# PaddlePaddle/PaddleFleetX

Measured on AMD Instinct MI355X. Metric: tokens/sec/GPU GPT-3-6.7B pretrain, DP2×TP2×PP2 at 1/2/4/8 MI355X, higher is better.
Workload: dtype bf16; 1 GPU; model=GPT-6.7B, global_batch=32, seq_len=1024, micro_batch=16, parallelism=dp1tp1pp1

## Files before the change

### csrc/bindings.cpp

```cpp
#include <torch/extension.h>

#include <string>
#include <vector>

std::vector<torch::Tensor> layernorm_fwd(torch::Tensor x, torch::Tensor w,
                                         torch::Tensor b, double eps);
std::vector<torch::Tensor> layernorm_bwd(torch::Tensor dy, torch::Tensor x,
                                         torch::Tensor w, torch::Tensor mean,
                                         torch::Tensor rstd);
std::vector<torch::Tensor> rmsnorm_fwd(torch::Tensor x, torch::Tensor w,
                                       double eps);
std::vector<torch::Tensor> rmsnorm_bwd(torch::Tensor dy, torch::Tensor x,
                                       torch::Tensor w, torch::Tensor rstd);
std::vector<torch::Tensor> layernorm_fwd_residual(torch::Tensor x,
                                                  torch::Tensor res,
                                                  torch::Tensor w,
                                                  torch::Tensor b, double eps);
std::vector<torch::Tensor> layernorm_bwd_residual(torch::Tensor dy,
                                                  torch::Tensor x,
                                                  torch::Tensor w,
                                                  torch::Tensor mean,
                                                  torch::Tensor rstd,
                                                  torch::Tensor dsum);
torch::Tensor bias_gelu_fwd(torch::Tensor x, torch::Tensor bias);
std::vector<torch::Tensor> bias_gelu_bwd(torch::Tensor dy, torch::Tensor x,
                                         torch::Tensor bias);
void adamw_flat(torch::Tensor master, torch::Tensor grad, torch::Tensor m,
                torch::Tensor v, torch::Tensor model, double lr, double beta1,
                double beta2, double eps, double wd, long step);
torch::Tensor rope_fwd(torch::Tensor x, torch::Tensor cos, torch::Tensor sin);
torch::Tensor colsum(torch::Tensor x);
void grad_sumsq(torch::Tensor x, torch::Tensor out, long slot);
torch::Tensor softmax_causal_fwd(torch::Tensor s, double scale);
torch::Tensor softmax_causal_bwd(torch::Tensor dy, torch::Tensor y,
                                 double scale);
torch::Tensor softmax_bias_fwd(torch::Tensor s, torch::Tensor bias,
                               long inner, long outer, double scale);
std::vector<torch::Tensor> cross_entropy_fwd(torch::Tensor logits,
// ... 44 lines not shown
                                       torch::Tensor sorted_idx,
                                       torch::Tensor top_p, torch::Tensor u);
std::vector<torch::Tensor> sample_token(
    torch::Tensor logits, torch::Tensor ids_buf, torch::Tensor lens,
    torch::Tensor unfinished, torch::Tensor u, torch::Tensor next_tokens,
    bool greedy, double temperature, long top_k, double top_p,
    double repetition_penalty, long min_length, long eos_token_id,
    long pad_token_id);
std::vector<torch::Tensor> moe_dispatch(torch::Tensor x,
                                        torch::Tensor expert_ids,
                                        long num_experts, long top_k);
torch::Tensor mfma_gemm16_probe(torch::Tensor a, torch::Tensor b);

PYBIND11_MODULE(TORCH_EXTENSION_NAME, m) {
  m.def("layernorm_fwd", &layernorm_fwd, "fused LayerNorm fwd (gfx950)");
  m.def("layernorm_bwd", &layernorm_bwd, "fused LayerNorm bwd");
  m.def("rmsnorm_fwd", &rmsnorm_fwd, "fused RMSNorm fwd");
  m.def("rmsnorm_bwd", &rmsnorm_bwd, "fused RMSNorm bwd");
  m.def("layernorm_fwd_residual", &layernorm_fwd_residual,
        "LN(a+b) fwd, also emits a+b");
  m.def("layernorm_bwd_residual", &layernorm_bwd_residual,
        "LN bwd with fused residual-grad addend");
  m.def("colsum", &colsum, "column sum [N,H] -> fp32 [H] (dbias)");
  m.def("grad_sumsq", &grad_sumsq, "fused sumsq (found_inf + grad norm)");
  m.def("bias_gelu_fwd", &bias_gelu_fwd, "fused bias+gelu fwd");
  m.def("bias_gelu_bwd", &bias_gelu_bwd, "fused bias+gelu bwd");
  m.def("adamw_flat", &adamw_flat, "fused AdamW on flat buffers");
  m.def("rope_fwd", &rope_fwd, "rotary embedding fwd");
  m.def("softmax_causal_fwd", &softmax_causal_fwd,
        "fused scale+causal-mask+softmax fwd");
  m.def("softmax_causal_bwd", &softmax_causal_bwd, "causal softmax bwd");
  m.def("softmax_bias_fwd", &softmax_bias_fwd,
        "fused scale+bias+softmax (gated attention core)");
  m.def("cross_entropy_fwd", &cross_entropy_fwd, "softmax CE fwd");
  m.def("cross_entropy_bwd", &cross_entropy_bwd, "softmax CE bwd");
  m.def("row_max", &row_max, "rowwise max (vocab-parallel CE)");
  m.def("row_sumexp", &row_sumexp, "rowwise sum(exp(x-m))");
// ... 60 lines not shown
```

### csrc/common.h

```cpp
#pragma once

#include <hip/hip_runtime.h>
#include <hip/hip_bf16.h>
#include <hip/hip_fp16.h>

#define WAVE 64
#define DEV_INLINE __device__ __forceinline__

typedef __attribute__((ext_vector_type(2))) short short2v;
typedef __attribute__((ext_vector_type(4))) short short4v;
typedef __attribute__((ext_vector_type(8))) short short8v;
typedef __attribute__((ext_vector_type(4))) float float4v;
typedef __attribute__((ext_vector_type(2))) float float2v;
typedef __attribute__((ext_vector_type(8))) __bf16 bf16x8;
typedef __attribute__((ext_vector_type(4))) __bf16 bf16x4;

typedef __attribute__((ext_vector_type(8))) __bf16 mfma_bf16x8;
typedef __attribute__((ext_vector_type(4))) float mfma_f32x4;

DEV_INLINE float bf2f(__hip_bfloat16 x) { return __bfloat162float(x); }
DEV_INLINE __hip_bfloat16 f2bf(float x) { return __float2bfloat16(x); }

DEV_INLINE float bf_raw2f(unsigned short u) {
  union { unsigned int i; float f; } v;
// ... 142 lines not shown
        ((unsigned short*)&out)[j + 1] = (unsigned short)(u >> 16);
      }
      *reinterpret_cast<short4v*>(p) = out;
    }
  } else {
#pragma unroll
    for (int j = 0; j < VEC; j += 4) {
      float4v out;
#pragma unroll
      for (int k = 0; k < 4; ++k) ((float*)&out)[k] = v[j + k];
      *reinterpret_cast<float4v*>((float*)p + j) = out;
    }
  }
}

#define HIP_CHECK(x)                                                       \
  do {                                                                     \
    hipError_t _e = (x);                                                   \
    if (_e != hipSuccess) {                                                \
      throw std::runtime_error(std::string("HIP error: ") +                \
                               hipGetErrorString(_e));                     \
    }                                                                      \
  } while (0)
```

### csrc/elementwise.hip

```cpp
#include "common.h"
#include "tensor_checks.h"

#include <torch/extension.h>
#include <ATen/hip/HIPContext.h>

namespace {

constexpr int BLOCK = 256;
constexpr float GELU_K = 0.7978845608028654f;

DEV_INLINE float fast_tanh(float y) {
  return 1.f - 2.f / (__expf(2.f * y) + 1.f);
}
DEV_INLINE float gelu_tanh(float x) {
  float t = fast_tanh(GELU_K * (x + 0.044715f * x * x * x));
  return 0.5f * x * (1.f + t);
}
DEV_INLINE float gelu_tanh_grad(float x) {
  float t = fast_tanh(GELU_K * (x + 0.044715f * x * x * x));
  return 0.5f * (1.f + t) +
         0.5f * x * (1.f - t * t) * GELU_K * (1.f + 3.f * 0.044715f * x * x);
}

template <typename T, bool HAS_BIAS, int VEC>
// ... 6 lines not shown
  if constexpr (HAS_BIAS) vload<T, VEC>(bias + col, bv);
  for (long r = blockIdx.y; r < N; r += gridDim.y) {
    const long i = r * H + col;
    float v[VEC];
    vload<T, VEC>(x + i, v);
    float o[VEC];
#pragma unroll
    for (int j = 0; j < VEC; ++j) {
      if constexpr (HAS_BIAS) v[j] += bv[j];
      o[j] = gelu_tanh(v[j]);
    }
    vstore<T, VEC>(y + i, o);
  }
}

template <typename T, bool HAS_BIAS, int VEC>
__global__ __launch_bounds__(BLOCK) void bias_gelu_bwd_kernel(
    const T* __restrict__ dy, const T* __restrict__ x,
    const T* __restrict__ bias, T* __restrict__ dx, long N, int H) {
  const int col = (blockIdx.x * BLOCK + threadIdx.x) * VEC;
  if (col >= H) return;
  float bv[VEC];
  if constexpr (HAS_BIAS) vload<T, VEC>(bias + col, bv);
  for (long r = blockIdx.y; r < N; r += gridDim.y) {
    const long i = r * H + col;
    float v[VEC], d[VEC];
    vload<T, VEC>(x + i, v);
    vload<T, VEC>(dy + i, d);
    float o[VEC];
#pragma unroll
    for (int j = 0; j < VEC; ++j) {
      if constexpr (HAS_BIAS) v[j] += bv[j];
      o[j] = d[j] * gelu_tanh_grad(v[j]);
    }
    vstore<T, VEC>(dx + i, o);
  }
}

template <typename T, int CV>
__global__ __launch_bounds__(BLOCK) void colsum_kernel(
    const T* __restrict__ x, float* __restrict__ out, long N, int H,
    int rows_per_chunk) {
  const int col = (blockIdx.x * BLOCK + threadIdx.x) * CV;
  if (col >= H) return;
  long r0 = (long)blockIdx.y * rows_per_chunk;
  long r1 = r0 + rows_per_chunk < N ? r0 + rows_per_chunk : N;
  float s[CV];
#pragma unroll
  for (int j = 0; j < CV; ++j) s[j] = 0.f;
  for (long r = r0; r < r1; ++r) {
    float v[CV];
    vload<T, CV>(x + r * H + col, v);
#pragma unroll
    for (int j = 0; j < CV; ++j) s[j] += v[j];
  }
#pragma unroll
  for (int j = 0; j < CV; ++j) atomicAdd(&out[col + j], s[j]);
}

template <typename T>
__global__ void grad_sumsq_kernel(const T* __restrict__ x, long n,
                                  float* __restrict__ partial) {
  __shared__ float sred[BLOCK / WAVE];
  float s = 0.f;
  constexpr int V = 4;
  for (long i = ((long)blockIdx.x * BLOCK + threadIdx.x) * V; i < n;
       i += (long)gridDim.x * BLOCK * V) {
    float v[V];
    vload<T, V>(x + i, v);
#pragma unroll
    for (int j = 0; j < V; ++j) s += v[j] * v[j];
  }
// ... 7 lines not shown
  __shared__ double sred[BLOCK / WAVE];
  double s = 0.0;
  for (int i = threadIdx.x; i < np; i += BLOCK) s += (double)partial[i];
#pragma unroll
  for (int off = 32; off > 0; off >>= 1) s += __shfl_xor(s, off, WAVE);
  if (threadIdx.x % WAVE == 0) sred[threadIdx.x / WAVE] = s;
  __syncthreads();
  if (threadIdx.x == 0) {
    double t = 0.0;
#pragma unroll
    for (int w = 0; w < BLOCK / WAVE; ++w) t += sred[w];
    out[slot] = (float)((double)out[slot] + t);
  }
}

void launch_colsum(const void* x, float* out, long N, int H, bool bf16,
                   hipStream_t stream) {
  constexpr int CV = 4;
  int rows_per_chunk = (int)std::max<long>(32, N / 128);
  int nchunks = (int)((N + rows_per_chunk - 1) / rows_per_chunk);
  dim3 grid((H + BLOCK * CV - 1) / (BLOCK * CV), nchunks);
  if (bf16)
    hipLaunchKernelGGL((colsum_kernel<__hip_bfloat16, CV>), grid, dim3(BLOCK),
                       0, stream, (const __hip_bfloat16*)x, out, N, H,
                       rows_per_chunk);
  else
    hipLaunchKernelGGL((colsum_kernel<float, CV>), grid, dim3(BLOCK), 0,
                       stream, (const float*)x, out, N, H, rows_per_chunk);
}

template <typename TM, typename TG>
__global__ void adamw_flat_kernel(float* __restrict__ master,
                                  const TG* __restrict__ grad,
                                  float* __restrict__ m, float* __restrict__ v,
                                  TM* __restrict__ model, long n, float lr,
                                  float beta1, float beta2, float eps,
                                  float wd, float bc1, float bc2) {
  const int VEC = 4;
  for (long i = ((long)blockIdx.x * BLOCK + threadIdx.x) * VEC; i < n;
       i += (long)gridDim.x * BLOCK * VEC) {
    float4v pm = *reinterpret_cast<float4v*>(master + i);
    float4v pg;
    if constexpr (sizeof(TG) == 2) {
// ... 116 lines not shown
                                         torch::Tensor bias) {
  fleetx::check_data(x, "x");
  TORCH_CHECK(x.dim() >= 1, "x must have a last dim");
  fleetx::check_same(dy, x, "dy");
  TORCH_CHECK(dy.sizes() == x.sizes(), "dy must have the shape of x");
  long total = x.numel();
  int H = x.size(-1);
  long N = total / H;
  TORCH_CHECK(H % 4 == 0, "last dim must be divisible by 4");
  bool has_bias = bias.defined() && bias.numel() > 0;
  if (has_bias) {
    fleetx::check_same(bias, x, "bias");
    fleetx::check_numel(bias, H, "bias");
  }
  auto dx = torch::empty_like(x);
  auto stream = at::hip::getCurrentHIPStream();
  bool v8 = H % 8 == 0;
  int vec = v8 ? 8 : 4;
  dim3 grid((H + BLOCK * vec - 1) / (BLOCK * vec),
            (unsigned)std::min<long>(N, 16384));
#define LAUNCH_BG(T, HB, V)                                                  \
  hipLaunchKernelGGL((bias_gelu_bwd_kernel<T, HB, V>), grid, dim3(BLOCK), 0, \
                     stream, (const T*)dy.data_ptr(), (const T*)x.data_ptr(), \
                     has_bias ? (const T*)bias.data_ptr() : nullptr,         \
                     (T*)dx.data_ptr(), N, H)
#define PICK_BG(T, HB) do { if (v8) LAUNCH_BG(T, HB, 8); else LAUNCH_BG(T, HB, 4); } while (0)
  if (x.scalar_type() == torch::kBFloat16) {
    if (has_bias) PICK_BG(__hip_bfloat16, true);
    else PICK_BG(__hip_bfloat16, false);
  } else {
    if (has_bias) PICK_BG(float, true);
    else PICK_BG(float, false);
  }
#undef PICK_BG
#undef LAUNCH_BG
  torch::Tensor db;
  if (has_bias) {
    db = torch::zeros({H}, x.options().dtype(torch::kFloat));
    launch_colsum(dx.data_ptr(), db.data_ptr<float>(), N, H,
                  x.scalar_type() == torch::kBFloat16, stream);
  }
  return {dx, db};
}

void grad_sumsq(torch::Tensor x, torch::Tensor out, long slot) {
  fleetx::check_data(x, "x");
  fleetx::check_aux(out, torch::kFloat, x, "out");
  TORCH_CHECK(slot >= 0 && slot < out.numel(), "slot ", slot,
              " is outside out (", out.numel(), " slots)");
  long n = x.numel();
  TORCH_CHECK(n % 4 == 0, "x.numel() must be divisible by 4");
  if (n == 0) return;
  auto stream = at::hip::getCurrentHIPStream();
  dim3 grid(grid_for(n, BLOCK * 4));
  auto partial = torch::empty({(long)grid.x}, out.options());
// ... 5 lines not shown
  else
    hipLaunchKernelGGL((grad_sumsq_kernel<float>), grid, dim3(BLOCK), 0,
                       stream, (const float*)x.data_ptr(), n,
                       partial.data_ptr<float>());
  hipLaunchKernelGGL(grad_sumsq_finish_kernel, dim3(1), dim3(BLOCK), 0,
                     stream, partial.data_ptr<float>(), (int)grid.x,
                     out.data_ptr<float>(), slot);
}

torch::Tensor colsum(torch::Tensor x) {
  fleetx::check_data(x, "x");
  TORCH_CHECK(x.dim() == 2, "x must be 2-D [N, H]");
  long N = x.size(0);
  int H = x.size(1);
  TORCH_CHECK(H % 4 == 0, "H must be divisible by 4");
  auto out = torch::zeros({H}, x.options().dtype(torch::kFloat));
  auto stream = at::hip::getCurrentHIPStream();
  launch_colsum(x.data_ptr(), out.data_ptr<float>(), N, H,
                x.scalar_type() == torch::kBFloat16, stream);
  return out;
}

void adamw_flat(torch::Tensor master, torch::Tensor grad, torch::Tensor m,
                torch::Tensor v, torch::Tensor model, double lr, double beta1,
                double beta2, double eps, double wd, long step) {
  TORCH_CHECK(master.is_cuda(), "master must be a GPU tensor");
  fleetx::check_aux(master, torch::kFloat, master, "master");
  long n = master.numel();
  TORCH_CHECK(n % 4 == 0, "master.numel() must be divisible by 4");
  fleetx::check_data(grad, "grad");
  TORCH_CHECK(grad.device() == master.device(), "grad is on ", grad.device(),
              ", expected ", master.device());
  fleetx::check_numel(grad, n, "grad");
  fleetx::check_aux(m, torch::kFloat, master, "m");
// ... 59 lines not shown
```

### csrc/layernorm.hip

```cpp
#include "common.h"
#include "tensor_checks.h"

#include <torch/extension.h>
#include <ATen/hip/HIPContext.h>

namespace {

constexpr int BLOCK = 256;

template <typename T, int VEC>
DEV_INLINE void load_vec(const T* p, float* v) {
  if constexpr (sizeof(T) == 2) {
    if constexpr (VEC == 8) {
      short8v pk = *reinterpret_cast<const short8v*>(p);
#pragma unroll
      for (int j = 0; j < 8; ++j) v[j] = bf_raw2f(((unsigned short*)&pk)[j]);
    } else {
      short4v pk = *reinterpret_cast<const short4v*>(p);
#pragma unroll
      for (int j = 0; j < 4; ++j) v[j] = bf_raw2f(((unsigned short*)&pk)[j]);
    }
  } else {
#pragma unroll
    for (int j = 0; j < VEC; j += 4) {
// ... 170 lines not shown
      if (b) {
        float bv[VEC];
        load_vec<T, VEC>(b + i, bv);
#pragma unroll
        for (int j = 0; j < VEC; ++j) o[j] = (v[j] - mu) * rs * wv[j] + bv[j];
      } else {
#pragma unroll
        for (int j = 0; j < VEC; ++j) o[j] = (v[j] - mu) * rs * wv[j];
      }
      store_vec<T, VEC>(yr + i, o);
    }
    __syncthreads();
  }
}

template <typename T, int VEC, int ITERS>
__global__ __launch_bounds__(BLOCK) void ln_bwd_dx_reg_kernel(
    const T* __restrict__ dy, const T* __restrict__ x,
    const T* __restrict__ w, const float* __restrict__ mean,
    const float* __restrict__ rstd, const T* __restrict__ dsum,
    T* __restrict__ dx, int N, int H, bool rms) {
  __shared__ float sred[BLOCK / WAVE];
  float wv[ITERS][VEC];
#pragma unroll
  for (int it = 0; it < ITERS; ++it)
    load_vec<T, VEC>(w + (it * BLOCK + threadIdx.x) * VEC, wv[it]);
  for (int row = blockIdx.x; row < N; row += gridDim.x) {
    const T* xr = x + (long)row * H;
    const T* dyr = dy + (long)row * H;
    float mu = rms ? 0.f : mean[row];
    float rs = rstd[row];
    float xh[ITERS][VEC], dw[ITERS][VEC];
    float c1 = 0.f, c2 = 0.f;
#pragma unroll
    for (int it = 0; it < ITERS; ++it) {
      int i = (it * BLOCK + threadIdx.x) * VEC;
      float xv[VEC], dv[VEC];
      load_vec<T, VEC>(xr + i, xv);
      load_vec<T, VEC>(dyr + i, dv);
#pragma unroll
      for (int j = 0; j < VEC; ++j) {
        xh[it][j] = (xv[j] - mu) * rs;
        dw[it][j] = dv[j] * wv[it][j];
        c1 += dw[it][j];
        c2 += dw[it][j] * xh[it][j];
      }
    }
    c1 = block_reduce_sum<BLOCK>(c1, sred) / H;
    __syncthreads();
    c2 = block_reduce_sum<BLOCK>(c2, sred) / H;
    T* dxr = dx + (long)row * H;
#pragma unroll
    for (int it = 0; it < ITERS; ++it) {
      int i = (it * BLOCK + threadIdx.x) * VEC;
      float o[VEC];
#pragma unroll
      for (int j = 0; j < VEC; ++j)
        o[j] = rms ? (dw[it][j] - xh[it][j] * c2) * rs
                   : (dw[it][j] - c1 - xh[it][j] * c2) * rs;
      if (dsum) {
        float av[VEC];
        load_vec<T, VEC>(dsum + (long)row * H + i, av);
#pragma unroll
        for (int j = 0; j < VEC; ++j) o[j] += av[j];
      }
      store_vec<T, VEC>(dxr + i, o);
    }
    __syncthreads();
  }
}

template <typename T, int VEC>
__global__ void ln_bwd_dx_kernel(const T* __restrict__ dy, const T* __restrict__ x,
                                 const T* __restrict__ w,
                                 const float* __restrict__ mean,
                                 const float* __restrict__ rstd,
                                 const T* __restrict__ dsum,
                                 T* __restrict__ dx, int N, int H, bool rms) {
  __shared__ float sred[BLOCK / WAVE];
  for (int row = blockIdx.x; row < N; row += gridDim.x) {
    const T* xr = x + (long)row * H;
    const T* dyr = dy + (long)row * H;
    float mu = rms ? 0.f : mean[row];
// ... 31 lines not shown
        float av[VEC];
        load_vec<T, VEC>(dsum + (long)row * H + i, av);
#pragma unroll
        for (int j = 0; j < VEC; ++j) o[j] += av[j];
      }
      store_vec<T, VEC>(dxr + i, o);
    }
    __syncthreads();
  }
}

template <typename T>
__global__ void ln_bwd_dwdb_kernel(const T* __restrict__ dy, const T* __restrict__ x,
                                   const float* __restrict__ mean,
                                   const float* __restrict__ rstd,
                                   float* __restrict__ dw, float* __restrict__ db,
                                   int N, int H, int rows_per_chunk, bool rms) {
  int col = blockIdx.x * BLOCK + threadIdx.x;
  if (col >= H) return;
  int r0 = blockIdx.y * rows_per_chunk;
  int r1 = min(N, r0 + rows_per_chunk);
  float sw = 0.f, sb = 0.f;
  for (int r = r0; r < r1; ++r) {
    float xv, dv;
    if constexpr (sizeof(T) == 2) {
      xv = bf_raw2f(((const unsigned short*)x)[(long)r * H + col]);
      dv = bf_raw2f(((const unsigned short*)dy)[(long)r * H + col]);
    } else {
      xv = ((const float*)x)[(long)r * H + col];
      dv = ((const float*)dy)[(long)r * H + col];
    }
    float mu = rms ? 0.f : mean[r];
    float xh = (xv - mu) * rstd[r];
    sw += dv * xh;
    sb += dv;
  }
  atomicAdd(&dw[col], sw);
  if (db) atomicAdd(&db[col], sb);
}

#define LN_FOR_EACH_SHAPE(F) \
  F(4, 1)      \
  F(8, 1)      \
  F(8, 2)      \
  F(4, 5)      \
  F(8, 4)

template <typename T>
void ln_fwd_launch(const T* x, const T* res, const T* w, const T* b, T* y,
                   T* sum_out, float* mean, float* rstd, int N, int H,
                   float eps, bool rms, hipStream_t stream) {
  int grid = std::min(N, 4096);
  TORCH_CHECK(H % 4 == 0, "hidden size must be divisible by 4");
// ... 4 lines not shown
                       mean, rstd, N, H, eps, rms);                         \
    return;                                                                 \
  }
  LN_FOR_EACH_SHAPE(LN_FWD_CASE)
#undef LN_FWD_CASE
  if (H % (8 * 4) == 0)
    hipLaunchKernelGGL((ln_fwd_kernel<T, 8>), dim3(grid), dim3(BLOCK), 0,
                       stream, x, res, w, b, y, sum_out, mean, rstd, N, H,
                       eps, rms);
  else
    hipLaunchKernelGGL((ln_fwd_kernel<T, 4>), dim3(grid), dim3(BLOCK), 0,
                       stream, x, res, w, b, y, sum_out, mean, rstd, N, H,
                       eps, rms);
}

template <typename T>
void ln_bwd_dx_launch(const T* dy, const T* x, const T* w, const float* mean,
                      const float* rstd, const T* dsum, T* dx, int N, int H,
                      bool rms, hipStream_t stream) {
  int grid = std::min(N, 4096);
#define LN_BWD_CASE(V, I)                                                   \
  if (H == BLOCK * V * I) {                                                 \
    hipLaunchKernelGGL((ln_bwd_dx_reg_kernel<T, V, I>), dim3(grid),         \
                       dim3(BLOCK), 0, stream, dy, x, w, mean, rstd, dsum,  \
                       dx, N, H, rms);                                      \
    return;                                                                 \
  }
  LN_FOR_EACH_SHAPE(LN_BWD_CASE)
#undef LN_BWD_CASE
  if (H % (8 * 4) == 0)
    hipLaunchKernelGGL((ln_bwd_dx_kernel<T, 8>), dim3(grid), dim3(BLOCK), 0,
                       stream, dy, x, w, mean, rstd, dsum, dx, N, H, rms);
  else
    hipLaunchKernelGGL((ln_bwd_dx_kernel<T, 4>), dim3(grid), dim3(BLOCK), 0,
                       stream, dy, x, w, mean, rstd, dsum, dx, N, H, rms);
}

}


static std::vector<torch::Tensor> ln_fwd_common(torch::Tensor x,
                                                c10::optional<torch::Tensor> res,
                                                torch::Tensor w,
                                                c10::optional<torch::Tensor> b,
                                                double eps, bool rms) {
  fleetx::check_data(x, "x");
  TORCH_CHECK(x.dim() == 2, "x must be 2-D [N, H]");
  int N = x.size(0), H = x.size(1);
  TORCH_CHECK(H % 4 == 0, "hidden size must be divisible by 4");
  fleetx::check_same(w, x, "w");
// ... 54 lines not shown
                                                  torch::Tensor b,
                                                  double eps) {
  return ln_fwd_common(x, res, w, b, eps, false);
}

std::vector<torch::Tensor> rmsnorm_fwd(torch::Tensor x, torch::Tensor w,
                                       double eps) {
  return ln_fwd_common(x, c10::nullopt, w, c10::nullopt, eps, true);
}

static std::vector<torch::Tensor> ln_bwd_impl(torch::Tensor dy, torch::Tensor x,
                                              torch::Tensor w,
                                              torch::Tensor mean_or_empty,
                                              torch::Tensor rstd,
                                              c10::optional<torch::Tensor> dsum,
                                              bool rms) {
  fleetx::check_data(x, "x");
  TORCH_CHECK(x.dim() == 2, "x must be 2-D [N, H]");
  int N = x.size(0), H = x.size(1);
  TORCH_CHECK(H % 4 == 0, "hidden size must be divisible by 4");
  fleetx::check_same(dy, x, "dy");
  TORCH_CHECK(dy.sizes() == x.sizes(), "dy must have the shape of x");
  fleetx::check_same(w, x, "w");
  fleetx::check_numel(w, H, "w");
  if (!rms) {
    fleetx::check_aux(mean_or_empty, torch::kFloat, x, "mean");
    fleetx::check_numel(mean_or_empty, N, "mean");
  }
  fleetx::check_aux(rstd, torch::kFloat, x, "rstd");
  fleetx::check_numel(rstd, N, "rstd");
  if (dsum.has_value()) {
    fleetx::check_same(*dsum, x, "dsum");
    TORCH_CHECK(dsum->sizes() == x.sizes(), "dsum must have the shape of x");
  }
  auto dx = torch::empty_like(x);
  auto dw = torch::zeros({H}, x.options().dtype(torch::kFloat));
  auto db = rms ? torch::Tensor()
                : torch::zeros({H}, x.options().dtype(torch::kFloat));
  auto stream = at::hip::getCurrentHIPStream();
  const float* mean_p = rms ? nullptr : mean_or_empty.data_ptr<float>();
  int rows_per_chunk = std::max(16, N / 256);
  int nchunks = (N + rows_per_chunk - 1) / rows_per_chunk;
  dim3 grid2((H + BLOCK - 1) / BLOCK, nchunks);
  if (x.scalar_type() == torch::kBFloat16) {
    using T = __hip_bfloat16;
    ln_bwd_dx_launch<T>((const T*)dy.data_ptr(), (const T*)x.data_ptr(),
                        (const T*)w.data_ptr(), mean_p,
                        rstd.data_ptr<float>(),
                        dsum.has_value() ? (const T*)dsum->data_ptr() : nullptr,
                        (T*)dx.data_ptr(), N, H, rms, stream);
    hipLaunchKernelGGL((ln_bwd_dwdb_kernel<T>), grid2, dim3(BLOCK), 0, stream,
                       (const T*)dy.data_ptr(), (const T*)x.data_ptr(), mean_p,
                       rstd.data_ptr<float>(), dw.data_ptr<float>(),
                       rms ? nullptr : db.data_ptr<float>(), N, H,
                       rows_per_chunk, rms);
  } else {
    ln_bwd_dx_launch<float>(dy.data_ptr<float>(), x.data_ptr<float>(),
                            w.data_ptr<float>(), mean_p,
                            rstd.data_ptr<float>(),
                            dsum.has_value() ? dsum->data_ptr<float>() : nullptr,
                            dx.data_ptr<float>(), N, H, rms, stream);
    hipLaunchKernelGGL((ln_bwd_dwdb_kernel<float>), grid2, dim3(BLOCK), 0,
                       stream, dy.data_ptr<float>(), x.data_ptr<float>(), mean_p,
                       rstd.data_ptr<float>(), dw.data_ptr<float>(),
                       rms ? nullptr : db.data_ptr<float>(), N, H,
                       rows_per_chunk, rms);
  }
  if (rms) return {dx, dw};
  return {dx, dw, db};
}

std::vector<torch::Tensor> layernorm_bwd(torch::Tensor dy, torch::Tensor x,
                                         torch::Tensor w, torch::Tensor mean,
                                         torch::Tensor rstd) {
  return ln_bwd_impl(dy, x, w, mean, rstd, c10::nullopt, false);
}

std::vector<torch::Tensor> layernorm_bwd_residual(torch::Tensor dy,
                                                  torch::Tensor x,
                                                  torch::Tensor w,
                                                  torch::Tensor mean,
                                                  torch::Tensor rstd,
                                                  torch::Tensor dsum) {
  return ln_bwd_impl(dy, x, w, mean, rstd, dsum, false);
}

std::vector<torch::Tensor> rmsnorm_bwd(torch::Tensor dy, torch::Tensor x,
                                       torch::Tensor w, torch::Tensor rstd) {
  return ln_bwd_impl(dy, x, w, torch::Tensor(), rstd, c10::nullopt, true);
}
```

### paddlefleetx_amd/ops/_reference.py

```python

from __future__ import annotations

import math
from typing import Optional, Tuple

import torch
import torch.nn.functional as F


def layernorm_fwd(x: torch.Tensor, weight: torch.Tensor, bias: torch.Tensor,
                  eps: float) -> Tuple[torch.Tensor, torch.Tensor, torch.Tensor]:
    xf = x.float()
    mean = xf.mean(dim=-1)
    var = xf.var(dim=-1, unbiased=False)
    rstd = torch.rsqrt(var + eps)
    y = (xf - mean[:, None]) * rstd[:, None] * weight.float() + bias.float()
    return y.to(x.dtype), mean, rstd


def layernorm_bwd(dy: torch.Tensor, x: torch.Tensor, weight: torch.Tensor,
                  mean: torch.Tensor, rstd: torch.Tensor
                  ) -> Tuple[torch.Tensor, torch.Tensor, torch.Tensor]:
    xf, dyf, wf = x.float(), dy.float(), weight.float()
    H = x.shape[-1]
    xhat = (xf - mean[:, None]) * rstd[:, None]
    dyw = dyf * wf
    c1 = dyw.mean(dim=-1, keepdim=True)
    c2 = (dyw * xhat).mean(dim=-1, keepdim=True)
    dx = (dyw - c1 - xhat * c2) * rstd[:, None]
    dw = (dyf * xhat).sum(dim=0)
    db = dyf.sum(dim=0)
    return dx.to(x.dtype), dw, db


def layernorm_fwd_residual(x: torch.Tensor, res: torch.Tensor,
                           weight: torch.Tensor, bias: torch.Tensor,
                           eps: float):
    s = (x.float() + res.float()).to(x.dtype)
    y, mean, rstd = layernorm_fwd(s, weight, bias, eps)
    return y, mean, rstd, s


def layernorm_bwd_residual(dy: torch.Tensor, s: torch.Tensor,
                           weight: torch.Tensor, mean: torch.Tensor,
                           rstd: torch.Tensor, dsum: torch.Tensor):
    dx, dw, db = layernorm_bwd(dy, s, weight, mean, rstd)
    dx = (dx.float() + dsum.float()).to(dx.dtype)
    return dx, dw, db


def rmsnorm_fwd(x: torch.Tensor, weight: torch.Tensor, eps: float
                ) -> Tuple[torch.Tensor, torch.Tensor]:
    xf = x.float()
    rstd = torch.rsqrt(xf.pow(2).mean(dim=-1) + eps)
    y = xf * rstd[:, None] * weight.float()
    return y.to(x.dtype), rstd


def rmsnorm_bwd(dy: torch.Tensor, x: torch.Tensor, weight: torch.Tensor,
                rstd: torch.Tensor) -> Tuple[torch.Tensor, torch.Tensor]:
    xf, dyf, wf = x.float(), dy.float(), weight.float()
    H = x.shape[-1]
    xhat = xf * rstd[:, None]
    dyw = dyf * wf
    c = (dyw * xhat).mean(dim=-1, keepdim=True)
    dx = (dyw - xhat * c) * rstd[:, None]
    dw = (dyf * xhat).sum(dim=0)
    return dx.to(x.dtype), dw


def bias_gelu_fwd(x: torch.Tensor, bias: Optional[torch.Tensor]) -> torch.Tensor:
    xf = x.float()
    if bias is not None:
        xf = xf + bias.float()
    y = 0.5 * xf * (1.0 + torch.tanh(0.7978845608028654 * (xf + 0.044715 * xf ** 3)))
    return y.to(x.dtype)


def bias_gelu_bwd(dy: torch.Tensor, x: torch.Tensor, bias: Optional[torch.Tensor]
                  ) -> Tuple[torch.Tensor, Optional[torch.Tensor]]:
    xf = x.float()
    if bias is not None:
        xf = xf + bias.float()
# ... 310 lines not shown
```

Measured before the change: 25860 tokens/s.

## Fuse column-sum reductions into LN and bias-GELU backward via deterministic partials

Replaces atomicAdd-based column sums with per-group fp32 partial buffers that a small finish kernel reduces in double. Bias-GELU backward now accumulates the bias gradient inside its main kernel instead of re-reading dx in a separate colsum pass. LayerNorm backward accumulates dw/db in registers within the dx kernel and can optionally emit the column sum of dx. The grid size is derived from occupancy, and the intent is to cut extra passes over activations and atomic contention, at the cost of extra launches, partial buffers and higher register pressure.

```diff
diff --git a/csrc/bindings.cpp b/csrc/bindings.cpp
--- a/csrc/bindings.cpp
+++ b/csrc/bindings.cpp
@@ -7,11 +7,12 @@
                                          torch::Tensor b, double eps);
 std::vector<torch::Tensor> layernorm_bwd(torch::Tensor dy, torch::Tensor x,
                                          torch::Tensor w, torch::Tensor mean,
-                                         torch::Tensor rstd);
+                                         torch::Tensor rstd, bool dcol);
 std::vector<torch::Tensor> rmsnorm_fwd(torch::Tensor x, torch::Tensor w,
                                        double eps);
 std::vector<torch::Tensor> rmsnorm_bwd(torch::Tensor dy, torch::Tensor x,
-                                       torch::Tensor w, torch::Tensor rstd);
+                                       torch::Tensor w, torch::Tensor rstd,
+                                       bool dcol);
 std::vector<torch::Tensor> layernorm_fwd_residual(torch::Tensor x,
                                                   torch::Tensor res,
                                                   torch::Tensor w,
@@ -21,7 +22,8 @@
                                                   torch::Tensor w,
                                                   torch::Tensor mean,
                                                   torch::Tensor rstd,
-                                                  torch::Tensor dsum);
+                                                  torch::Tensor dsum,
+                                                  bool dcol);
 torch::Tensor bias_gelu_fwd(torch::Tensor x, torch::Tensor bias);
 std::vector<torch::Tensor> bias_gelu_bwd(torch::Tensor dy, torch::Tensor x,
                                          torch::Tensor bias);
@@ -96,13 +98,22 @@
 
 PYBIND11_MODULE(TORCH_EXTENSION_NAME, m) {
   m.def("layernorm_fwd", &layernorm_fwd, "fused LayerNorm fwd (gfx950)");
-  m.def("layernorm_bwd", &layernorm_bwd, "fused LayerNorm bwd");
+  m.def("layernorm_bwd", &layernorm_bwd,
+        "fused LayerNorm bwd -> (dx, dw, db[, dcol]); dcol=True appends the "
+        "fp32 column sum of the returned dx",
+        py::arg("dy"), py::arg("x"), py::arg("w"), py::arg("mean"),
+        py::arg("rstd"), py::arg("dcol") = false);
   m.def("rmsnorm_fwd", &rmsnorm_fwd, "fused RMSNorm fwd");
-  m.def("rmsnorm_bwd", &rmsnorm_bwd, "fused RMSNorm bwd");
+  m.def("rmsnorm_bwd", &rmsnorm_bwd,
+        "fused RMSNorm bwd -> (dx, dw[, dcol])",
+        py::arg("dy"), py::arg("x"), py::arg("w"), py::arg("rstd"),
+        py::arg("dcol") = false);
   m.def("layernorm_fwd_residual", &layernorm_fwd_residual,
         "LN(a+b) fwd, also emits a+b");
   m.def("layernorm_bwd_residual", &layernorm_bwd_residual,
-        "LN bwd with fused residual-grad addend");
+        "LN bwd with fused residual-grad addend -> (dx, dw, db[, dcol])",
+        py::arg("dy"), py::arg("x"), py::arg("w"), py::arg("mean"),
+        py::arg("rstd"), py::arg("dsum"), py::arg("dcol") = false);
   m.def("colsum", &colsum, "column sum [N,H] -> fp32 [H] (dbias)");
   m.def("grad_sumsq", &grad_sumsq, "fused sumsq (found_inf + grad norm)");
   m.def("bias_gelu_fwd", &bias_gelu_fwd, "fused bias+gelu fwd");
diff --git a/csrc/column_partials.h b/csrc/column_partials.h
--- /dev/null
+++ b/csrc/column_partials.h
@@ -0,0 +1,77 @@
+#pragma once
+
+#include "common.h"
+
+#include <algorithm>
+#include <stdexcept>
+#include <string>
+
+namespace fleetx {
+
+constexpr int CP_MAX_ROWS = 128;
+constexpr int CP_MIN_ROWS = 32;
+
+inline int cp_groups(long N, long col_blocks, long resident_blocks) {
+  long fit = std::max<long>(1, resident_blocks / std::max<long>(1, col_blocks));
+  long most = (N + CP_MIN_ROWS - 1) / CP_MIN_ROWS;
+  long least = (N + CP_MAX_ROWS - 1) / CP_MAX_ROWS;
+  return (int)std::max<long>(least, std::min<long>(fit, most));
+}
+
+inline long cp_resident_blocks(const void* kernel, int block) {
+  int per_cu = 0, dev = 0, cus = 0;
+  HIP_CHECK(hipOccupancyMaxActiveBlocksPerMultiprocessor(&per_cu, kernel,
+                                                         block, 0));
+  HIP_CHECK(hipGetDevice(&dev));
+  HIP_CHECK(hipDeviceGetAttribute(&cus, hipDeviceAttributeMultiprocessorCount,
+                                  dev));
+  return (long)std::max(1, per_cu) * std::max(1, cus);
+}
+
+constexpr int CP_FIN_BLOCK = 256;
+constexpr int CP_FIN_COLT = 8;
+constexpr int CP_FIN_SLICES = CP_FIN_BLOCK / CP_FIN_COLT;
+constexpr int CP_FIN_COLS = CP_FIN_COLT * 4;
+
+static __global__ __launch_bounds__(CP_FIN_BLOCK) void colsum_finish_kernel(
+    const float* __restrict__ partial, int groups, int H,
+    float* __restrict__ out0, float* __restrict__ out1,
+    float* __restrict__ out2) {
+  __shared__ double sred[CP_FIN_SLICES][CP_FIN_COLS];
+  const int ct = threadIdx.x % CP_FIN_COLT;
+  const int sl = threadIdx.x / CP_FIN_COLT;
+  const int col = (blockIdx.x * CP_FIN_COLT + ct) * 4;
+  const float* p = partial + (long)blockIdx.y * groups * H;
+  double s[4] = {0.0, 0.0, 0.0, 0.0};
+  if (col < H) {
+#pragma unroll 4
+    for (int g = sl; g < groups; g += CP_FIN_SLICES) {
+      float4v v = *reinterpret_cast<const float4v*>(p + (long)g * H + col);
+#pragma unroll
+      for (int k = 0; k < 4; ++k) s[k] += (double)((float*)&v)[k];
+    }
+  }
+#pragma unroll
+  for (int k = 0; k < 4; ++k) sred[sl][ct * 4 + k] = s[k];
+  __syncthreads();
+  if (threadIdx.x < CP_FIN_COLS) {
+    const int c = blockIdx.x * CP_FIN_COLS + threadIdx.x;
+    if (c < H) {
+      double t = 0.0;
+#pragma unroll
+      for (int i = 0; i < CP_FIN_SLICES; ++i) t += sred[i][threadIdx.x];
+      float* out = blockIdx.y == 0 ? out0 : (blockIdx.y == 1 ? out1 : out2);
+      out[c] = (float)t;
+    }
+  }
+}
+
+inline void launch_colsum_finish(const float* partial, int nvec, int groups,
+                                 int H, float* out0, float* out1, float* out2,
+                                 hipStream_t stream) {
+  dim3 grid((H + CP_FIN_COLS - 1) / CP_FIN_COLS, nvec);
+  hipLaunchKernelGGL(colsum_finish_kernel, grid, dim3(CP_FIN_BLOCK), 0, stream,
+                     partial, groups, H, out0, out1, out2);
+}
+
+}
diff --git a/csrc/common.h b/csrc/common.h
--- a/csrc/common.h
+++ b/csrc/common.h
@@ -180,7 +180,19 @@
   }
 }
 
-#define HIP_CHECK(x)                                                       \
+template <typename T, int VEC>
+DEV_INLINE void round_io(float* v) {
+  if constexpr (sizeof(T) == 2) {
+#pragma unroll
+    for (int j = 0; j < VEC; j += 2) {
+      unsigned int u = cvt_pk_bf16(v[j], v[j + 1]);
+      v[j] = bf_raw2f((unsigned short)u);
+      v[j + 1] = bf_raw2f((unsigned short)(u >> 16));
+    }
+  }
+}
+
+#define HIP_CHECK(x)                                                      \
   do {                                                                     \
     hipError_t _e = (x);                                                   \
     if (_e != hipSuccess) {                                                \
diff --git a/csrc/elementwise.hip b/csrc/elementwise.hip
--- a/csrc/elementwise.hip
+++ b/csrc/elementwise.hip
@@ -1,4 +1,5 @@
 #include "common.h"
+#include "column_partials.h"
 #include "tensor_checks.h"
 
 #include <torch/extension.h>
@@ -44,14 +45,19 @@
   }
 }
 
+#define BG_BWD_MIN_WAVES(T, HAS_BIAS) (sizeof(T) == 2 || (HAS_BIAS) ? 8 : 1)
 template <typename T, bool HAS_BIAS, int VEC>
-__global__ __launch_bounds__(BLOCK) void bias_gelu_bwd_kernel(
+__global__ __launch_bounds__(BLOCK, BG_BWD_MIN_WAVES(T, HAS_BIAS))
+void bias_gelu_bwd_kernel(
     const T* __restrict__ dy, const T* __restrict__ x,
-    const T* __restrict__ bias, T* __restrict__ dx, long N, int H) {
+    const T* __restrict__ bias, T* __restrict__ dx,
+    float* __restrict__ db_partial, long N, int H) {
   const int col = (blockIdx.x * BLOCK + threadIdx.x) * VEC;
   if (col >= H) return;
-  float bv[VEC];
+  float bv[VEC], s[VEC];
   if constexpr (HAS_BIAS) vload<T, VEC>(bias + col, bv);
+#pragma unroll
+  for (int j = 0; j < VEC; ++j) s[j] = 0.f;
   for (long r = blockIdx.y; r < N; r += gridDim.y) {
     const long i = r * H + col;
     float v[VEC], d[VEC];
@@ -63,29 +69,46 @@
       if constexpr (HAS_BIAS) v[j] += bv[j];
       o[j] = d[j] * gelu_tanh_grad(v[j]);
     }
+    if constexpr (HAS_BIAS) {
+      round_io<T, VEC>(o);
+#pragma unroll
+      for (int j = 0; j < VEC; ++j) {
+#pragma clang fp contract(off)
+        s[j] += o[j];
+      }
+    }
     vstore<T, VEC>(dx + i, o);
   }
+  if constexpr (HAS_BIAS)
+    vstore<float, VEC>(db_partial + (long)blockIdx.y * H + col, s);
 }
 
 template <typename T, int CV>
 __global__ __launch_bounds__(BLOCK) void colsum_kernel(
-    const T* __restrict__ x, float* __restrict__ out, long N, int H,
-    int rows_per_chunk) {
+    const T* __restrict__ x, float* __restrict__ partial, long N, int H) {
   const int col = (blockIdx.x * BLOCK + threadIdx.x) * CV;
   if (col >= H) return;
-  long r0 = (long)blockIdx.y * rows_per_chunk;
-  long r1 = r0 + rows_per_chunk < N ? r0 + rows_per_chunk : N;
   float s[CV];
 #pragma unroll
   for (int j = 0; j < CV; ++j) s[j] = 0.f;
-  for (long r = r0; r < r1; ++r) {
+  const long G = gridDim.y;
+  long r = blockIdx.y;
+  for (; r + 3 * G < N; r += 4 * G) {
+    float v[4][CV];
+#pragma unroll
+    for (int k = 0; k < 4; ++k) vload<T, CV>(x + (r + k * G) * H + col, v[k]);
+#pragma unroll
+    for (int k = 0; k < 4; ++k)
+#pragma unroll
+      for (int j = 0; j < CV; ++j) s[j] += v[k][j];
+  }
+  for (; r < N; r += G) {
     float v[CV];
     vload<T, CV>(x + r * H + col, v);
 #pragma unroll
     for (int j = 0; j < CV; ++j) s[j] += v[j];
   }
-#pragma unroll
-  for (int j = 0; j < CV; ++j) atomicAdd(&out[col + j], s[j]);
+  vstore<float, CV>(partial + (long)blockIdx.y * H + col, s);
 }
 
 template <typename T>
@@ -123,19 +146,26 @@
   }
 }
 
-void launch_colsum(const void* x, float* out, long N, int H, bool bf16,
+void launch_colsum(const torch::Tensor& x, float* out, long N, int H,
                    hipStream_t stream) {
-  constexpr int CV = 4;
-  int rows_per_chunk = (int)std::max<long>(32, N / 128);
-  int nchunks = (int)((N + rows_per_chunk - 1) / rows_per_chunk);
-  dim3 grid((H + BLOCK * CV - 1) / (BLOCK * CV), nchunks);
-  if (bf16)
-    hipLaunchKernelGGL((colsum_kernel<__hip_bfloat16, CV>), grid, dim3(BLOCK),
-                       0, stream, (const __hip_bfloat16*)x, out, N, H,
-                       rows_per_chunk);
-  else
-    hipLaunchKernelGGL((colsum_kernel<float, CV>), grid, dim3(BLOCK), 0,
-                       stream, (const float*)x, out, N, H, rows_per_chunk);
+  const bool bf16 = x.scalar_type() == torch::kBFloat16;
+  const int cv = bf16 && H % 8 == 0 ? 8 : 4;
+  const void* kfn =
+      !bf16 ? (const void*)&colsum_kernel<float, 4>
+            : (cv == 8 ? (const void*)&colsum_kernel<__hip_bfloat16, 8>
+                       : (const void*)&colsum_kernel<__hip_bfloat16, 4>);
+  dim3 grid((H + BLOCK * cv - 1) / (BLOCK * cv));
+  const int groups =
+      fleetx::cp_groups(N, grid.x, fleetx::cp_resident_blocks(kfn, BLOCK));
+  grid.y = groups;
+  auto partial = torch::empty({(long)groups, (long)H},
+                              x.options().dtype(torch::kFloat));
+  float* pp = partial.data_ptr<float>();
+  const void* xp = x.data_ptr();
+  void* args[] = {&xp, &pp, &N, &H};
+  HIP_CHECK(hipLaunchKernel(kfn, grid, dim3(BLOCK), args, 0, stream));
+  fleetx::launch_colsum_finish(pp, 1, groups, H, out, nullptr, nullptr,
+                               stream);
 }
 
 template <typename TM, typename TG>
@@ -282,17 +312,18 @@
     fleetx::check_numel(bias, H, "bias");
   }
   auto dx = torch::empty_like(x);
+  torch::Tensor db;
+  if (N == 0) {
+    if (has_bias) db = torch::zeros({H}, x.options().dtype(torch::kFloat));
+    return {dx, db};
+  }
   auto stream = at::hip::getCurrentHIPStream();
   bool v8 = H % 8 == 0;
   int vec = v8 ? 8 : 4;
-  dim3 grid((H + BLOCK * vec - 1) / (BLOCK * vec),
-            (unsigned)std::min<long>(N, 16384));
-#define LAUNCH_BG(T, HB, V)                                                  \
-  hipLaunchKernelGGL((bias_gelu_bwd_kernel<T, HB, V>), grid, dim3(BLOCK), 0, \
-                     stream, (const T*)dy.data_ptr(), (const T*)x.data_ptr(), \
-                     has_bias ? (const T*)bias.data_ptr() : nullptr,         \
-                     (T*)dx.data_ptr(), N, H)
-#define PICK_BG(T, HB) do { if (v8) LAUNCH_BG(T, HB, 8); else LAUNCH_BG(T, HB, 4); } while (0)
+  const void* kfn;
+#define PICK_BG(T, HB) \
+  kfn = v8 ? (const void*)&bias_gelu_bwd_kernel<T, HB, 8> \
+           : (const void*)&bias_gelu_bwd_kernel<T, HB, 4>
   if (x.scalar_type() == torch::kBFloat16) {
     if (has_bias) PICK_BG(__hip_bfloat16, true);
     else PICK_BG(__hip_bfloat16, false);
@@ -301,12 +332,25 @@
     else PICK_BG(float, false);
   }
 #undef PICK_BG
-#undef LAUNCH_BG
-  torch::Tensor db;
+  dim3 grid((H + BLOCK * vec - 1) / (BLOCK * vec));
+  const int groups =
+      fleetx::cp_groups(N, grid.x, fleetx::cp_resident_blocks(kfn, BLOCK));
+  grid.y = groups;
+  torch::Tensor partial;
+  if (has_bias)
+    partial = torch::empty({(long)groups, (long)H},
+                           x.options().dtype(torch::kFloat));
+  float* pp = has_bias ? partial.data_ptr<float>() : nullptr;
+  const void* dyp = dy.data_ptr();
+  const void* xp = x.data_ptr();
+  const void* bp = has_bias ? bias.data_ptr() : nullptr;
+  void* dxp = dx.data_ptr();
+  void* args[] = {&dyp, &xp, &bp, &dxp, &pp, &N, &H};
+  HIP_CHECK(hipLaunchKernel(kfn, grid, dim3(BLOCK), args, 0, stream));
   if (has_bias) {
-    db = torch::zeros({H}, x.options().dtype(torch::kFloat));
-    launch_colsum(dx.data_ptr(), db.data_ptr<float>(), N, H,
-                  x.scalar_type() == torch::kBFloat16, stream);
+    db = torch::empty({H}, x.options().dtype(torch::kFloat));
+    fleetx::launch_colsum_finish(pp, 1, groups, H, db.data_ptr<float>(),
+                                 nullptr, nullptr, stream);
   }
   return {dx, db};
 }
@@ -342,10 +386,10 @@
   long N = x.size(0);
   int H = x.size(1);
   TORCH_CHECK(H % 4 == 0, "H must be divisible by 4");
-  auto out = torch::zeros({H}, x.options().dtype(torch::kFloat));
-  auto stream = at::hip::getCurrentHIPStream();
-  launch_colsum(x.data_ptr(), out.data_ptr<float>(), N, H,
-                x.scalar_type() == torch::kBFloat16, stream);
+  if (N == 0) return torch::zeros({H}, x.options().dtype(torch::kFloat));
+  auto out = torch::empty({H}, x.options().dtype(torch::kFloat));
+  auto stream = at::hip::getCurrentHIPStream();
+  launch_colsum(x, out.data_ptr<float>(), N, H, stream);
   return out;
 }
 
diff --git a/csrc/layernorm.hip b/csrc/layernorm.hip
--- a/csrc/layernorm.hip
+++ b/csrc/layernorm.hip
@@ -1,4 +1,5 @@
 #include "common.h"
+#include "column_partials.h"
 #include "tensor_checks.h"
 
 #include <torch/extension.h>
@@ -208,17 +209,25 @@
   }
 }
 
-template <typename T, int VEC, int ITERS>
+template <typename T, int VEC, int ITERS, bool DCOL>
 __global__ __launch_bounds__(BLOCK) void ln_bwd_dx_reg_kernel(
     const T* __restrict__ dy, const T* __restrict__ x,
     const T* __restrict__ w, const float* __restrict__ mean,
     const float* __restrict__ rstd, const T* __restrict__ dsum,
-    T* __restrict__ dx, int N, int H, bool rms) {
+    T* __restrict__ dx, float* __restrict__ part, int N, int H, bool rms) {
   __shared__ float sred[BLOCK / WAVE];
   float wv[ITERS][VEC];
-#pragma unroll
-  for (int it = 0; it < ITERS; ++it)
+  float gw[ITERS][VEC], gb[ITERS][VEC], gc[DCOL ? ITERS : 1][VEC];
+#pragma unroll
+  for (int it = 0; it < ITERS; ++it) {
     load_vec<T, VEC>(w + (it * BLOCK + threadIdx.x) * VEC, wv[it]);
+#pragma unroll
+    for (int j = 0; j < VEC; ++j) {
+      gw[it][j] = 0.f;
+      gb[it][j] = 0.f;
+      if constexpr (DCOL) gc[it][j] = 0.f;
+    }
+  }
   for (int row = blockIdx.x; row < N; row += gridDim.x) {
     const T* xr = x + (long)row * H;
     const T* dyr = dy + (long)row * H;
@@ -238,6 +247,8 @@
         dw[it][j] = dv[j] * wv[it][j];
         c1 += dw[it][j];
         c2 += dw[it][j] * xh[it][j];
+        gw[it][j] += dv[j] * xh[it][j];
+        gb[it][j] += dv[j];
       }
     }
     c1 = block_reduce_sum<BLOCK>(c1, sred) / H;
@@ -258,9 +269,22 @@
 #pragma unroll
         for (int j = 0; j < VEC; ++j) o[j] += av[j];
       }
+      if constexpr (DCOL) {
+        round_io<T, VEC>(o);
+#pragma unroll
+        for (int j = 0; j < VEC; ++j) gc[it][j] += o[j];
+      }
       store_vec<T, VEC>(dxr + i, o);
     }
     __syncthreads();
+  }
+  const long gh = (long)gridDim.x * H;
+#pragma unroll
+  for (int it = 0; it < ITERS; ++it) {
+    float* p = part + (long)blockIdx.x * H + (it * BLOCK + threadIdx.x) * VEC;
+    store_vec<float, VEC>(p, gw[it]);
+    if (!rms) store_vec<float, VEC>(p + gh, gb[it]);
+    if constexpr (DCOL) store_vec<float, VEC>(p + (rms ? gh : 2 * gh), gc[it]);
   }
 }
 
@@ -322,29 +346,35 @@
 __global__ void ln_bwd_dwdb_kernel(const T* __restrict__ dy, const T* __restrict__ x,
                                    const float* __restrict__ mean,
                                    const float* __restrict__ rstd,
-                                   float* __restrict__ dw, float* __restrict__ db,
+                                   const T* __restrict__ dxs,
+                                   float* __restrict__ part,
                                    int N, int H, int rows_per_chunk, bool rms) {
   int col = blockIdx.x * BLOCK + threadIdx.x;
   if (col >= H) return;
   int r0 = blockIdx.y * rows_per_chunk;
   int r1 = min(N, r0 + rows_per_chunk);
-  float sw = 0.f, sb = 0.f;
+  float sw = 0.f, sb = 0.f, sc = 0.f;
   for (int r = r0; r < r1; ++r) {
     float xv, dv;
     if constexpr (sizeof(T) == 2) {
       xv = bf_raw2f(((const unsigned short*)x)[(long)r * H + col]);
       dv = bf_raw2f(((const unsigned short*)dy)[(long)r * H + col]);
+      if (dxs) sc += bf_raw2f(((const unsigned short*)dxs)[(long)r * H + col]);
     } else {
       xv = ((const float*)x)[(long)r * H + col];
       dv = ((const float*)dy)[(long)r * H + col];
+      if (dxs) sc += ((const float*)dxs)[(long)r * H + col];
     }
     float mu = rms ? 0.f : mean[r];
     float xh = (xv - mu) * rstd[r];
     sw += dv * xh;
     sb += dv;
   }
-  atomicAdd(&dw[col], sw);
-  if (db) atomicAdd(&db[col], sb);
+  const long gh = (long)gridDim.y * H;
+  float* p = part + (long)blockIdx.y * H + col;
+  p[0] = sw;
+  if (!rms) p[gh] = sb;
+  if (dxs) p[rms ? gh : 2 * gh] = sc;
 }
 
 #define LN_FOR_EACH_SHAPE(F) \
@@ -379,26 +409,59 @@
                        eps, rms);
 }
 
+constexpr int LN_BWD_GRID = 1024;
+
 template <typename T>
-void ln_bwd_dx_launch(const T* dy, const T* x, const T* w, const float* mean,
-                      const float* rstd, const T* dsum, T* dx, int N, int H,
-                      bool rms, hipStream_t stream) {
+const void* ln_bwd_reg_fn(int H, bool dcol) {
+#define LN_FN_CASE(V, I)                                                \
+  if (H == BLOCK * V * I)                                               \
+    return dcol ? (const void*)&ln_bwd_dx_reg_kernel<T, V, I, true>     \
+                : (const void*)&ln_bwd_dx_reg_kernel<T, V, I, false>;
+  LN_FOR_EACH_SHAPE(LN_FN_CASE)
+#undef LN_FN_CASE
+  return nullptr;
+}
+
+int ln_bwd_reg_grid(const void* fn, int N) {
+  int need = (N + fleetx::CP_MAX_ROWS - 1) / fleetx::CP_MAX_ROWS;
+  int fit = (int)std::min<long>(LN_BWD_GRID,
+                                fleetx::cp_resident_blocks(fn, BLOCK));
+  return std::min(N, std::max(fit, need));
+}
+
+int ln_bwd_chunk_rows(int N) {
+  return std::min(fleetx::CP_MAX_ROWS, std::max(16, N / 256));
+}
+
+template <typename T>
+int ln_bwd_groups(int N, int H, bool dcol) {
+  if (const void* fn = ln_bwd_reg_fn<T>(H, dcol)) return ln_bwd_reg_grid(fn, N);
+  int rows_per_chunk = ln_bwd_chunk_rows(N);
+  return (N + rows_per_chunk - 1) / rows_per_chunk;
+}
+
+template <typename T>
+void ln_bwd_launch(const T* dy, const T* x, const T* w, const float* mean,
+                   const float* rstd, const T* dsum, T* dx, float* part,
+                   int groups, bool dcol, int N, int H, bool rms,
+                   hipStream_t stream) {
+  if (const void* fn = ln_bwd_reg_fn<T>(H, dcol)) {
+    void* args[] = {&dy, &x, &w, &mean, &rstd, &dsum, &dx, &part, &N, &H, &rms};
+    HIP_CHECK(hipLaunchKernel(fn, dim3(groups), dim3(BLOCK), args, 0, stream));
+    return;
+  }
   int grid = std::min(N, 4096);
-#define LN_BWD_CASE(V, I)                                                   \
-  if (H == BLOCK * V * I) {                                                 \
-    hipLaunchKernelGGL((ln_bwd_dx_reg_kernel<T, V, I>), dim3(grid),         \
-                       dim3(BLOCK), 0, stream, dy, x, w, mean, rstd, dsum,  \
-                       dx, N, H, rms);                                      \
-    return;                                                                 \
-  }
-  LN_FOR_EACH_SHAPE(LN_BWD_CASE)
-#undef LN_BWD_CASE
   if (H % (8 * 4) == 0)
     hipLaunchKernelGGL((ln_bwd_dx_kernel<T, 8>), dim3(grid), dim3(BLOCK), 0,
                        stream, dy, x, w, mean, rstd, dsum, dx, N, H, rms);
   else
     hipLaunchKernelGGL((ln_bwd_dx_kernel<T, 4>), dim3(grid), dim3(BLOCK), 0,
                        stream, dy, x, w, mean, rstd, dsum, dx, N, H, rms);
+  int rows_per_chunk = ln_bwd_chunk_rows(N);
+  dim3 grid2((H + BLOCK - 1) / BLOCK, groups);
+  hipLaunchKernelGGL((ln_bwd_dwdb_kernel<T>), grid2, dim3(BLOCK), 0, stream,
+                     dy, x, mean, rstd, dcol ? (const T*)dx : nullptr, part,
+                     N, H, rows_per_chunk, rms);
 }
 
 }
@@ -483,7 +546,7 @@
                                               torch::Tensor mean_or_empty,
                                               torch::Tensor rstd,
                                               c10::optional<torch::Tensor> dsum,
-                                              bool rms) {
+                                              bool rms, bool want_dcol) {
   fleetx::check_data(x, "x");
   TORCH_CHECK(x.dim() == 2, "x must be 2-D [N, H]");
   int N = x.size(0), H = x.size(1);
@@ -503,46 +566,45 @@
     TORCH_CHECK(dsum->sizes() == x.sizes(), "dsum must have the shape of x");
   }
   auto dx = torch::empty_like(x);
-  auto dw = torch::zeros({H}, x.options().dtype(torch::kFloat));
-  auto db = rms ? torch::Tensor()
-                : torch::zeros({H}, x.options().dtype(torch::kFloat));
+  auto fopt = x.options().dtype(torch::kFloat);
+  std::vector<torch::Tensor> out{dx};
+  const int nvec = (rms ? 1 : 2) + (want_dcol ? 1 : 0);
+  if (N == 0) {
+    for (int v = 0; v < nvec; ++v) out.push_back(torch::zeros({H}, fopt));
+    return out;
+  }
+  for (int v = 0; v < nvec; ++v) out.push_back(torch::empty({H}, fopt));
   auto stream = at::hip::getCurrentHIPStream();
   const float* mean_p = rms ? nullptr : mean_or_empty.data_ptr<float>();
-  int rows_per_chunk = std::max(16, N / 256);
-  int nchunks = (N + rows_per_chunk - 1) / rows_per_chunk;
-  dim3 grid2((H + BLOCK - 1) / BLOCK, nchunks);
-  if (x.scalar_type() == torch::kBFloat16) {
+  const bool bf16 = x.scalar_type() == torch::kBFloat16;
+  const int groups = bf16 ? ln_bwd_groups<__hip_bfloat16>(N, H, want_dcol)
+                          : ln_bwd_groups<float>(N, H, want_dcol);
+  auto part = torch::empty({(long)nvec, (long)groups, (long)H}, fopt);
+  if (bf16) {
     using T = __hip_bfloat16;
-    ln_bwd_dx_launch<T>((const T*)dy.data_ptr(), (const T*)x.data_ptr(),
-                        (const T*)w.data_ptr(), mean_p,
-                        rstd.data_ptr<float>(),
-                        dsum.has_value() ? (const T*)dsum->data_ptr() : nullptr,
-                        (T*)dx.data_ptr(), N, H, rms, stream);
-    hipLaunchKernelGGL((ln_bwd_dwdb_kernel<T>), grid2, dim3(BLOCK), 0, stream,
-                       (const T*)dy.data_ptr(), (const T*)x.data_ptr(), mean_p,
-                       rstd.data_ptr<float>(), dw.data_ptr<float>(),
-                       rms ? nullptr : db.data_ptr<float>(), N, H,
-                       rows_per_chunk, rms);
+    ln_bwd_launch<T>((const T*)dy.data_ptr(), (const T*)x.data_ptr(),
+                     (const T*)w.data_ptr(), mean_p, rstd.data_ptr<float>(),
+                     dsum.has_value() ? (const T*)dsum->data_ptr() : nullptr,
+                     (T*)dx.data_ptr(), part.data_ptr<float>(), groups,
+                     want_dcol, N, H, rms, stream);
   } else {
-    ln_bwd_dx_launch<float>(dy.data_ptr<float>(), x.data_ptr<float>(),
-                            w.data_ptr<float>(), mean_p,
-                            rstd.data_ptr<float>(),
-                            dsum.has_value() ? dsum->data_ptr<float>() : nullptr,
-                            dx.data_ptr<float>(), N, H, rms, stream);
-    hipLaunchKernelGGL((ln_bwd_dwdb_kernel<float>), grid2, dim3(BLOCK), 0,
-                       stream, dy.data_ptr<float>(), x.data_ptr<float>(), mean_p,
-                       rstd.data_ptr<float>(), dw.data_ptr<float>(),
-                       rms ? nullptr : db.data_ptr<float>(), N, H,
-                       rows_per_chunk, rms);
-  }
-  if (rms) return {dx, dw};
-  return {dx, dw, db};
+    ln_bwd_launch<float>(dy.data_ptr<float>(), x.data_ptr<float>(),
+                         w.data_ptr<float>(), mean_p, rstd.data_ptr<float>(),
+                         dsum.has_value() ? dsum->data_ptr<float>() : nullptr,
+                         dx.data_ptr<float>(), part.data_ptr<float>(), groups,
+                         want_dcol, N, H, rms, stream);
+  }
+  fleetx::launch_colsum_finish(
+      part.data_ptr<float>(), nvec, groups, H, out[1].data_ptr<float>(),
+      nvec > 1 ? out[2].data_ptr<float>() : nullptr,
+      nvec > 2 ? out[3].data_ptr<float>() : nullptr, stream);
+  return out;
 }
 
 std::vector<torch::Tensor> layernorm_bwd(torch::Tensor dy, torch::Tensor x,
                                          torch::Tensor w, torch::Tensor mean,
-                                         torch::Tensor rstd) {
-  return ln_bwd_impl(dy, x, w, mean, rstd, c10::nullopt, false);
+                                         torch::Tensor rstd, bool dcol) {
+  return ln_bwd_impl(dy, x, w, mean, rstd, c10::nullopt, false, dcol);
 }
 
 std::vector<torch::Tensor> layernorm_bwd_residual(torch::Tensor dy,
@@ -550,11 +612,14 @@
                                                   torch::Tensor w,
                                                   torch::Tensor mean,
                                                   torch::Tensor rstd,
-                                                  torch::Tensor dsum) {
-  return ln_bwd_impl(dy, x, w, mean, rstd, dsum, false);
+                                                  torch::Tensor dsum,
+                                                  bool dcol) {
+  return ln_bwd_impl(dy, x, w, mean, rstd, dsum, false, dcol);
 }
 
 std::vector<torch::Tensor> rmsnorm_bwd(torch::Tensor dy, torch::Tensor x,
-                                       torch::Tensor w, torch::Tensor rstd) {
-  return ln_bwd_impl(dy, x, w, torch::Tensor(), rstd, c10::nullopt, true);
-}
+                                       torch::Tensor w, torch::Tensor rstd,
+                                       bool dcol) {
+  return ln_bwd_impl(dy, x, w, torch::Tensor(), rstd, c10::nullopt, true,
+                     dcol);
+}
diff --git a/paddlefleetx_amd/ops/_reference.py b/paddlefleetx_amd/ops/_reference.py
--- a/paddlefleetx_amd/ops/_reference.py
+++ b/paddlefleetx_amd/ops/_reference.py
@@ -18,9 +18,14 @@
     return y.to(x.dtype), mean, rstd
 
 
+def _with_dcol(dx: torch.Tensor, rest: tuple, dcol: bool) -> tuple:
+    if not dcol:
+        return (dx,) + rest
+    return (dx,) + rest + (dx.float().sum(dim=0),)
+
+
 def layernorm_bwd(dy: torch.Tensor, x: torch.Tensor, weight: torch.Tensor,
-                  mean: torch.Tensor, rstd: torch.Tensor
-                  ) -> Tuple[torch.Tensor, torch.Tensor, torch.Tensor]:
+                  mean: torch.Tensor, rstd: torch.Tensor, dcol: bool = False):
     xf, dyf, wf = x.float(), dy.float(), weight.float()
     H = x.shape[-1]
     xhat = (xf - mean[:, None]) * rstd[:, None]
@@ -30,7 +35,7 @@
     dx = (dyw - c1 - xhat * c2) * rstd[:, None]
     dw = (dyf * xhat).sum(dim=0)
     db = dyf.sum(dim=0)
-    return dx.to(x.dtype), dw, db
+    return _with_dcol(dx.to(x.dtype), (dw, db), dcol)
 
 
 def layernorm_fwd_residual(x: torch.Tensor, res: torch.Tensor,
@@ -43,10 +48,11 @@
 
 def layernorm_bwd_residual(dy: torch.Tensor, s: torch.Tensor,
                            weight: torch.Tensor, mean: torch.Tensor,
-                           rstd: torch.Tensor, dsum: torch.Tensor):
+                           rstd: torch.Tensor, dsum: torch.Tensor,
+                           dcol: bool = False):
     dx, dw, db = layernorm_bwd(dy, s, weight, mean, rstd)
     dx = (dx.float() + dsum.float()).to(dx.dtype)
-    return dx, dw, db
+    return _with_dcol(dx, (dw, db), dcol)
 
 
 def rmsnorm_fwd(x: torch.Tensor, weight: torch.Tensor, eps: float
@@ -58,7 +64,7 @@
 
 
 def rmsnorm_bwd(dy: torch.Tensor, x: torch.Tensor, weight: torch.Tensor,
-                rstd: torch.Tensor) -> Tuple[torch.Tensor, torch.Tensor]:
+                rstd: torch.Tensor, dcol: bool = False):
     xf, dyf, wf = x.float(), dy.float(), weight.float()
     H = x.shape[-1]
     xhat = xf * rstd[:, None]
@@ -66,7 +72,7 @@
     c = (dyw * xhat).mean(dim=-1, keepdim=True)
     dx = (dyw - xhat * c) * rstd[:, None]
     dw = (dyf * xhat).sum(dim=0)
-    return dx.to(x.dtype), dw
+    return _with_dcol(dx.to(x.dtype), (dw,), dcol)
 
 
 def bias_gelu_fwd(x: torch.Tensor, bias: Optional[torch.Tensor]) -> torch.Tensor:
```

Result: faster. 26320 tokens/s, median of 3 (+1.8%).
